# matwilso/generative_models

Measured on AMD Instinct MI355X. Metric: ddpm_train_images_per_sec, higher is better.
Workload: dtype fp16_fwd+bf16_bwd; 1 GPU; DDPM train step, 3x32x32, SimpleUnet C=128, 2048 images per GPU, T=1000 (BASELINE.json configs[2]); key=cfg2, global_batch=2048, parallelism=dp1

## Files before the change

generative_models_amd/csrc/conv1x1_stream.hip:

```cpp
#include <type_traits>

#include "gmk_common.h"

namespace {

constexpr int kRow = 272;

template <typename T>
__global__ __launch_bounds__(256) void conv1x1_pair_stream_kernel(const T* __restrict__ src, const T* __restrict__ w, T* __restrict__ out_a,
                                                                 T* __restrict__ out_b, unsigned npix, unsigned ntiles, unsigned src_bytes) {
    fp16_saturating_stores<T>();
    typedef typename Frag16<T>::type frag_t;
    typedef __attribute__((ext_vector_type(4))) unsigned int u32x4s;
    constexpr unsigned kBadOff = 0xFFFFFF00u;
    __shared__ __attribute__((aligned(16))) char wl[256 * kRow];
    __shared__ __attribute__((aligned(16))) char tile[128 * kRow];
    __shared__ __attribute__((aligned(16))) char trans[4 * 32 * kRow];
    const int tid = threadIdx.x, lane = tid & 63, wave = tid >> 6;
    const int r = lane & 31, h = lane >> 5;
    const __amdgpu_buffer_rsrc_t rss = __builtin_amdgcn_make_buffer_rsrc(const_cast<T*>(src), 0, (int)src_bytes, 0x00020000);
    const __amdgpu_buffer_rsrc_t rsa = __builtin_amdgcn_make_buffer_rsrc(out_a, 0, (int)src_bytes, 0x00020000);
    const __amdgpu_buffer_rsrc_t rsb = __builtin_amdgcn_make_buffer_rsrc(out_b, 0, (int)src_bytes, 0x00020000);
#pragma unroll
    for (int i = 0; i < 16; ++i) {
// ... 145 lines not shown
                s16x4 hi = __builtin_amdgcn_ds_read_tr16_b64_v4i16((GMK_LDS s16x4*)(Yb + (pxl + 4) * 256 + wa));
                const s16x8 t = {lo[0], lo[1], lo[2], lo[3], hi[0], hi[1], hi[2], hi[3]};
                a[i] = __builtin_bit_cast(bf16x8, t);
                lo = __builtin_amdgcn_ds_read_tr16_b64_v4i16((GMK_LDS s16x4*)(Xb + pxl * 256 + wb));
                hi = __builtin_amdgcn_ds_read_tr16_b64_v4i16((GMK_LDS s16x4*)(Xb + (pxl + 4) * 256 + wb));
                const s16x8 u = {lo[0], lo[1], lo[2], lo[3], hi[0], hi[1], hi[2], hi[3]};
                b[i] = __builtin_bit_cast(bf16x8, u);
            }
#pragma unroll
            for (int i = 0; i < 2; ++i)
#pragma unroll
                for (int j = 0; j < 2; ++j) acc[i][j] = __builtin_amdgcn_mfma_f32_32x32x16_bf16(a[i], b[j], acc[i][j], 0, 0, 0);
        }
        if (ks + 1 < nk) write_step(PAR ^ 1, ry[PAR ^ 1], rx0[PAR ^ 1], rx1[PAR ^ 1]);
        __syncthreads();
    };
    for (int ks = 0; ks < nk; ks += 2) {
        k_step(ks, std::integral_constant<int, 0>{});
        if (ks + 1 < nk) k_step(ks + 1, std::integral_constant<int, 1>{});
    }
    float* out = slab + (int64_t)blockIdx.x * (128 * 256) + cib * 128;
#pragma unroll
    for (int i = 0; i < 2; ++i)
#pragma unroll
        for (int j = 0; j < 2; ++j)
#pragma unroll
            for (int e = 0; e < 16; ++e) {
                const int co = wm * 64 + i * 32 + (e & 3) + 8 * (e >> 2) + 4 * h;
                const int ci = wn * 64 + j * 32 + r;
                out[co * 256 + ci] = acc[i][j][e];
            }
}

}

int gmk_conv1x1_pair_stream_try(const void* src, int64_t npix, const void* w_rows256, void* out_a, void* out_b, int dtype, hipStream_t stream) {
    if (!gmk_is16(dtype) || gmk_kernel_choice(3, "GMK_DEV_VARIANT") == 46) return 0;
    const int64_t bytes = npix * 256;
    if (bytes >= 0xFFFFFF00ll) return 0;
    const int64_t ntiles = (npix + 127) / 128;
    const int ncu = gmk_cu_limit();
    if (ntiles < 2 * ncu) return 0;
    const unsigned grid = (unsigned)ncu;
    if (dtype == GMK_BF16)
        conv1x1_pair_stream_kernel<bf16_t><<<grid, 256, 0, stream>>>((const bf16_t*)src, (const bf16_t*)w_rows256, (bf16_t*)out_a, (bf16_t*)out_b,
                                                                    (unsigned)npix, (unsigned)ntiles, (unsigned)bytes);
    else
        conv1x1_pair_stream_kernel<f16_t><<<grid, 256, 0, stream>>>((const f16_t*)src, (const f16_t*)w_rows256, (f16_t*)out_a, (f16_t*)out_b,
                                                                   (unsigned)npix, (unsigned)ntiles, (unsigned)bytes);
    return 1;
}

int gmk_conv1x1_wgrad_stream_try(const void* dy, int dy_cstride, const void* src0, const void* src1, int64_t npix, float* slab, int64_t slab_bytes,
                                 bool x_f16, hipStream_t stream) {
    if (gmk_kernel_choice(3, "GMK_DEV_VARIANT") == 47) return 0;
    const int ncu = gmk_cu_limit();
    if (npix < (int64_t)ncu * 64 * 8 || npix >= (1ll << 31) - 64) return 0;
    if (slab_bytes < (int64_t)ncu * 128 * 256 * 4) return 0;
    int64_t chunk = (npix + ncu - 1) / ncu;
    chunk = (chunk + 63) / 64 * 64;
    const int ns = (int)((npix + chunk - 1) / chunk);
    if (x_f16)
        conv1x1_wgrad_stream_kernel<f16_t><<<ns, 512, 0, stream>>>((const bf16_t*)dy, dy_cstride, (const f16_t*)src0, (const f16_t*)src1, slab, (int)npix, (int)chunk);
    else
        conv1x1_wgrad_stream_kernel<bf16_t><<<ns, 512, 0, stream>>>((const bf16_t*)dy, dy_cstride, (const bf16_t*)src0, (const bf16_t*)src1, slab, (int)npix, (int)chunk);
    return ns;
}
```

generative_models_amd/csrc/conv_igemm.hip:

```cpp
#include <stdlib.h>

#include <type_traits>

#include "gmk_common.h"

namespace {

constexpr int kBM = 128, kBN = 128;

struct GatherParams {
    int hs, ws;
    int ho, wo;
    int ksize, pad;
    int mul, shift, mask, lim_h, lim_w;
    signed char ty[9], tx[9];
    unsigned char tapw[9];
    int ntaps;
    int oscale, ooy, oox, out_w, out_hw;
};

__host__ bool make_gather(int mode, int ksize, int hs, int ws, int ho, int wo, GatherParams* g) {
    g->hs = hs; g->ws = ws; g->ho = ho; g->wo = wo;
    g->ksize = ksize; g->pad = ksize == 3 ? 1 : 0;
    g->mul = 1; g->shift = 0; g->mask = 0; g->lim_h = hs; g->lim_w = ws;
// ... 1120 lines not shown
            return gmk_check_launch("gmk_conv_wgrad(reduce)");
        }
    }
    if (wforce != 1 && ksize == 1 && mode == GMK_CONV_NORMAL && dtype == GMK_BF16 && c0 == 128 && c1 == 128 && cout == 128) {
        const int ns1 = gmk_conv1x1_wgrad_stream_try(dy, dy_cstride, src0, src1, (int64_t)B * ho * wo, (float*)workspace, workspace_bytes, xf16,
                                                     gmk_stream(stream));
        if (ns1 > 0) {
            gmk_note_kernel(15);
            int rc1 = gmk_check_launch("gmk_conv_wgrad(1x1 stream)");
            if (rc1) return rc1;
            launch_wgrad_reduce((const float*)workspace, dw, ns1, 1, cout, 256, gmk_stream(stream));
            return gmk_check_launch("gmk_conv_wgrad(reduce)");
        }
    }
    p.dy = dy; p.dy_cstride = dy_cstride; p.src0 = src0; p.src1 = src1; p.c0 = c0; p.c1 = c1; p.ktot = c0 + c1;
    p.cout = cout; p.M = B * ho * wo;
    const int ns = wgrad_nsplit(p.M, taps, cout, p.ktot, &p.chunk);
    const int64_t need = (int64_t)ns * taps * cout * p.ktot * 4;
    GMK_REQUIRE(workspace_bytes >= need, "gmk_conv_wgrad: workspace %lld < %lld bytes", (long long)workspace_bytes,
                (long long)need);
    p.slab = (float*)workspace;
    gmk_note_kernel(11);
    p.ns = ns; p.taps = taps; p.order = (gmk_kernel_choice(3, "GMK_DEV_VARIANT") & 0xFF) == 61;
    dim3 grid((ns + 7) / 8 * 8 * taps * (cout / 128) * (p.ktot / 128));
    if (dtype == GMK_BF16 && xf16) conv_wgrad_kernel<bf16_t, f16_t><<<grid, 256, 0, gmk_stream(stream)>>>(p);
    else if (dtype == GMK_BF16) conv_wgrad_kernel<bf16_t><<<grid, 256, 0, gmk_stream(stream)>>>(p);
    else if (fp32_split()) conv_wgrad_kernel<float, float, true><<<grid, 256, 0, gmk_stream(stream)>>>(p);
    else conv_wgrad_kernel<float><<<grid, 256, 0, gmk_stream(stream)>>>(p);
    int rc = gmk_check_launch("gmk_conv_wgrad");
    if (rc) return rc;
    launch_wgrad_reduce(p.slab, dw, ns, taps, cout, p.ktot, gmk_stream(stream));
    return gmk_check_launch("gmk_conv_wgrad(reduce)");
}
```

generative_models_amd/csrc/gmk_common.h:

```cpp
#pragma once
#include <hip/hip_runtime.h>
#include <stdint.h>

#include <type_traits>

#include "../../include/gmk.h"

typedef __bf16 bf16_t;
typedef __attribute__((ext_vector_type(8))) __bf16 bf16x8;
typedef __attribute__((ext_vector_type(4))) __bf16 bf16x4;
typedef _Float16 f16_t;
typedef __attribute__((ext_vector_type(8))) _Float16 f16x8;
typedef __attribute__((ext_vector_type(4))) _Float16 f16x4;
typedef __attribute__((ext_vector_type(2))) _Float16 f16x2;
typedef __attribute__((ext_vector_type(2))) __bf16 bf16x2;
typedef __attribute__((ext_vector_type(4))) short s16x4;
typedef __attribute__((ext_vector_type(4))) float f32x4;
typedef __attribute__((ext_vector_type(16))) float f32x16;

#define GMK_LDS __attribute__((address_space(3)))

void gmk_set_error(const char* fmt, ...);
int gmk_check_launch(const char* what);
int gmk_kernel_choice(int which, const char* env);
int gmk_conv1x1_pair_stream_try(const void* src, int64_t npix, const void* w_rows256, void* out_a, void* out_b, int dtype, hipStream_t stream);
int gmk_conv1x1_wgrad_stream_try(const void* dy, int dy_cstride, const void* src0, const void* src1, int64_t npix, float* slab, int64_t slab_bytes,
                                 bool x_f16, hipStream_t stream);
int gmk_conv_subpixel_takes(int B, int H, int W, int cin, int cout, int w_rows, int ntaps, int out_cstride, int dtype);
bool fp32_split(void);
int gmk_cu_limit(void);
void gmk_note_kernel(int id);

#define GMK_REQUIRE(cond, ...)                 \
    do {                                       \
        if (!(cond)) {                         \
            gmk_set_error(__VA_ARGS__);        \
            return GMK_ERR_ARG;                \
        }                                      \
    } while (0)

int gmk_conv3x3_halo_try(const void* src0, const void* src1, int c0, int c1, int B, int H, int W, const void* w, int w_rows,
                         int n0, int cout, const float* bias, const float* emb, int emb_stride, const void* residual,
                         void* out, int out_cstride, int min_tiles, int upsample, float* stats, int64_t stats_bytes,
                         const float* gn_scale, const float* gn_shift, int gn_stride, int dtype, hipStream_t stream);

struct HaloGeometry { int R, TP, slots; int64_t rows_total, M, ntiles, nb0, nb1, nbw, nbo; };
int gmk_halo_geometry(int B, int H, int W, int c0, int c1, int w_rows, int cout, int out_cstride, int min_tiles, int upsample,
                      int fused_gn, HaloGeometry* g);

int gmk_wgrad_slots_nsplit(int cout, int ktot);
int gmk_conv_wgrad_slots_try(const void* dy, int dy_cstride, const void* src0, const void* src1, int c0, int c1, int B, int H,
                             int W, int cout, float* slab, int64_t slab_bytes, int forced, int upsample, bool x_f16,
                             hipStream_t stream, int stride2 = 0);


static inline hipStream_t gmk_stream(void* s) { return reinterpret_cast<hipStream_t>(s); }
static inline int gmk_esize(int dtype) { return dtype == GMK_F32 ? 4 : 2; }
static inline bool gmk_is16(int dtype) { return dtype == GMK_BF16 || dtype == GMK_F16; }
template <typename T> struct gmk_tag { typedef T type; };
template <typename T> constexpr int gmk_dtype_of = std::is_same<T, float>::value ? GMK_F32 : std::is_same<T, bf16_t>::value ? GMK_BF16 : GMK_F16;
// ... 150 lines not shown
```

generative_models_amd/diffusion/simple_unet.py:

```python
import math
import os
from collections import OrderedDict

import torch
from torch import nn

from .. import ops

MAX_TIMESTEPS = 256


def _res_names(prefix, cin, cout, emb):
    out = [
        (f"{prefix}.in_layers.0.weight", (cin,)), (f"{prefix}.in_layers.0.bias", (cin,)),
        (f"{prefix}.in_layers.2.weight", (cout, cin, 3, 3)), (f"{prefix}.in_layers.2.bias", (cout,)),
        (f"{prefix}.emb_layers.1.weight", (cout, emb)), (f"{prefix}.emb_layers.1.bias", (cout,)),
        (f"{prefix}.out_layers.0.weight", (cout,)), (f"{prefix}.out_layers.0.bias", (cout,)),
        (f"{prefix}.out_layers.3.weight", (cout, cout, 3, 3)), (f"{prefix}.out_layers.3.bias", (cout,)),
    ]
    if cin != cout:
        out += [(f"{prefix}.skip_connection.weight", (cout, cin, 1, 1)), (f"{prefix}.skip_connection.bias", (cout,))]
    return out


# ... 538 lines not shown
                ops.set_cu_limit(part[0] - part[1])
        for t in tensors:
            t.record_stream(side)

    def _emb_ready(self):
        pend = getattr(self, "_emb_pending", None)
        if pend is not None:
            self._emb_pending = None
            self._join_side()
            pend.record_stream(torch.cuda.current_stream())

    def _join_side(self):
        if self._side is not None:
            torch.cuda.current_stream().wait_stream(self._side)

    def _res_bwd(self, name, ctx, dout, dout_sum, demb_all, blk, extra_add=None, grads=True, defer_skip=False):
        P, G, C = self._pv, self._gv, self.channels
        srcs, a, stats1, h, a2, (mean2, rstd2) = ctx.pop(name)
        B, H, W, _ = dout.shape
        two = len(srcs) == 2
        if grads:
            ops.colsum(dout_sum, G[f"{name}.out_layers.3.bias"], defer=True)
            self._wgrad(dout, [a2], 3, ops.NORMAL, G[f"{name}.out_layers.3.weight"])
        _, wd2 = self._packs[f"{name}.out_layers.3"]
        da2 = self._conv([dout], wd2, C, 3, ops.NORMAL, (H, W))
        dh, dgp, dbp = ops.gn_silu_bwd(da2, h, P[f"{name}.out_layers.0.weight"], P[f"{name}.out_layers.0.bias"], mean2,
                                       rstd2, dxsum=demb_all[:, blk * C:(blk + 1) * C] if grads else None,
                                       dropout=ctx.pop(name + ".dropout", None), xadd=ctx["emb_all"][:, blk * C:(blk + 1) * C])
        if grads:
            ops.colsum(dgp, G[f"{name}.out_layers.0.weight"], defer=True); ops.colsum(dbp, G[f"{name}.out_layers.0.bias"], defer=True)
            ops.colsum(demb_all[:, blk * C:(blk + 1) * C], G[f"{name}.in_layers.2.bias"], defer=True)
            self._wgrad(dh, a, 3, ops.NORMAL, G[f"{name}.in_layers.2.weight"])
        _, wd1 = self._packs[f"{name}.in_layers.2"]
        if two:
            if grads:
                ops.colsum(dout_sum, G[f"{name}.skip_connection.bias"], defer=True)
                self._wgrad(dout, srcs, 1, ops.NORMAL, G[f"{name}.skip_connection.weight"])
            _, wds = self._packs[f"{name}.skip_connection"]
        outs = []
        gw, gb = G[f"{name}.in_layers.0.weight"], G[f"{name}.in_layers.0.bias"]
        if two and C == 128:
            dskips = ops.conv1x1_pair(dout, wds, 2 * C)
        elif two:
            dskips = tuple(self._conv([dout], wds, 2 * C, 1, ops.NORMAL, (H, W), n0=i * C) for i in range(2))
        else:
            dskips = (dout,)
        for i, s in enumerate(srcs):
            da = self._conv([dh], wd1, len(srcs) * C, 3, ops.NORMAL, (H, W), n0=i * C)
            dskip = dskips[i]
            add2 = extra_add[i] if extra_add is not None else None
            gn = (da, dskip, P[f"{name}.in_layers.0.weight"][i * C:(i + 1) * C], P[f"{name}.in_layers.0.bias"][i * C:(i + 1) * C],
                  stats1[i][0], stats1[i][1])
            if defer_skip and i == 1 and grads and C == 128 and not self._narrow and ops.gn_pair_ok(s, self._g2, self._g1, da.dtype):
                outs.append((_DeferredGN(s, gn, gw[C:2 * C], gb[C:2 * C]), None))
                continue
            ssum = torch.empty((B, C), device=dout.device, dtype=torch.float32) if grads else None
            if isinstance(add2, _DeferredGN):
                assert add2.x is s
                ds, (ugp, ubp), (dgp, dbp) = ops.gn_silu_bwd_pair(s, add2.gn, gn, dxsum=ssum)
                ops.colsum(ugp, add2.gw, defer=True); ops.colsum(ubp, add2.gb, defer=True)
            else:
                ds, dgp, dbp = ops.gn_silu_bwd(da, s, *gn[2:], dadd1=dskip, dadd2=add2, dxsum=ssum)
            if grads:
                ops.colsum(dgp, gw[i * C:(i + 1) * C], defer=True); ops.colsum(dbp, gb[i * C:(i + 1) * C], defer=True)
            outs.append((ds, ssum))
        return outs

    def prepare_forward(self, dev=None):
        if self._packs_stale or self._packed_version != self._version_sum():
            self._repack()
        dev = self.flat_params.device if dev is None else dev
        self._freq_table(MAX_TIMESTEPS, dev)
        self._freq_table(4, dev)

# ... 189 lines not shown
```

generative_models_amd/ops.py:

```python
import math

import os

import torch

from ._lib import check, lib

F32, BF16, F16 = 0, 1, 2
_DT = {torch.float32: F32, torch.bfloat16: BF16, torch.float16: F16}
_HALF = (torch.bfloat16, torch.float16)
NORMAL, STRIDE2, UPSAMPLE2, TRANSPOSED2 = 0, 1, 2, 3

PROFILE = None


KERNEL_NAMES = {1: "conv_igemm_kernel", 2: "conv_igemm_dma_kernel", 3: "conv3x3_halo_kernel", 4: "conv3x3_halo_ws_kernel", 11: "conv_wgrad_kernel",
                12: "conv_wgrad_slots_kernel", 13: "conv_wgrad_slots_ws_kernel", 16: "conv_wgrad_subpixel_ws_kernel", 14: "conv1x1_pair_stream_kernel", 15: "conv1x1_wgrad_stream_kernel",
                5: "conv3x3_halo_ws_kernel[zero-stuffed transposed conv]",
                7: "conv3x3_halo_ws_kernel[+1x1 skip]",
                6: "conv_igemm_dma_kernel[stride-2 dgrad phases]",
                17: "conv_wgrad_slots_ws_kernel[stride-2 planes]",
                8: "conv_subpixel_ws_kernel[upsample]", 9: "conv_subpixel_ws_kernel[transposed]", 10: "conv_subpixel_ws_kernel[upsample dgrad]",
                21: "gn_silu_fwd_reg_kernel", 22: "gn_silu_fwd_kernel", 23: "gn_silu_bwd_hybrid_kernel", 24: "gn_silu_bwd_kernel",
                25: "gn_silu_bwd_pair_kernel", 26: "gn_silu_fwd_pair_kernel"}


def instantiation_key(name, dtype):
    if dtype not in _HALF:
        return None
    t = "f16" if dtype == torch.float16 else "bf16"
    if name == "conv3x3_halo_ws_kernel":
        return f"{name}<{t}>"
    if name == "conv3x3_halo_ws_kernel[+1x1 skip]":
        return f"conv3x3_halo_ws_kernel<{t},+skip>"
    if name == "conv_wgrad_slots_ws_kernel[stride-2 planes]":
        return "conv_wgrad_slots_ws_kernel<stride-2 planes>"
    if name.startswith("conv_subpixel_ws_kernel["):
        return f"conv_subpixel_ws_kernel<{t},{name[len('conv_subpixel_ws_kernel['):-1]}>"
    return None


def _nbytes(*tensors):
    if PROFILE is None:
        return 0.0
    return float(sum(t.numel() * t.element_size() for t in tensors if t is not None))


class _Timed:

    def __init__(self, name, flops, nbytes=0.0, fixed=False, multiplied=None, dtype=None):
# ... 88 lines not shown
    _f32(w, "w")
    cout, cin, k, _ = w.shape
    ref = w_fwd if w_fwd is not None else w_dgrad
    for t in (w_fwd, w_dgrad):
        if t is not None:
            _chk(t, name="pack")
            assert t.numel() == w.numel()
    if w_fwd is not None and w_dgrad is not None and w_fwd.dtype != w_dgrad.dtype:
        pack_conv_weight(w, w_fwd, None)
        pack_conv_weight(w, None, w_dgrad)
        return
    check(lib.gmk_pack_conv_weight(_p(w), _p(w_fwd), _p(w_dgrad), cout, cin, k, _DT[ref.dtype], _s()), "pack_conv_weight")


def pack_conv_weights_multi(arena, packs, table, fwd_f16=None):
    import ctypes
    _f32(arena, "arena"); _chk(packs, name="packs")
    n = len(table[0])
    arrs = [(ctypes.c_int * n)(*[int(v) for v in col]) for col in table]
    flags = (ctypes.c_int * n)(*[int(v) for v in fwd_f16]) if fwd_f16 is not None else None
    check(lib.gmk_pack_conv_weights_multi(_p(arena), _p(packs), n, *arrs, flags, _DT[packs.dtype], _s()), "pack_conv_weights_multi")


GN_STATS = False
GN_FUSE = os.environ.get("GMK_GN_FUSE", "1") != "0"
GN_FUSE_MIN_HW = int(os.environ.get("GMK_GN_FUSE_MIN_HW", "2048"))
SKIP_FOLD = os.environ.get("GMK_SKIP_FOLD", "1") != "0"
SKIP_FOLD_OVER_FUSE = os.environ.get("GMK_SKIP_FOLD_FUSE", "fold") != "fuse"
EMB_SIDE = os.environ.get("GMK_EMB_SIDE", "1") == "1"
FWD_SIDE = os.environ.get("GMK_FWD_SIDE", "0") == "1"
WGRAD_CUS = int(os.environ.get("GMK_WGRAD_CUS", "0"))
WGRAD_STREAM = os.environ.get("GMK_WGRAD_STREAM", "1") != "0"
GN_PAIR = os.environ.get("GMK_GN_PAIR", "1") != "0"


def _xadd_stride(xadd, B, C):
    if xadd is None:
        return 0
    assert xadd.dtype == torch.float32 and xadd.shape == (B, C) and xadd.stride(1) == 1 and xadd.is_cuda
    return xadd.stride(0)


def gn_silu_fwd(x, gamma, beta, groups, eps=1e-5, dropout=None, xadd=None):
    _chk(x, name="x"); _f32(gamma, "gamma"); _f32(beta, "beta")
    B, H, W, C = x.shape
    assert gamma.numel() == C and beta.numel() == C
    y = torch.empty_like(x)
    ncol = groups if groups > 0 else (C - groups - 1) // -groups
    mean = torch.empty((B, ncol), device=x.device, dtype=torch.float32)
    rstd = torch.empty_like(mean)
    mean._gn_groups = groups
    st = getattr(x, "_gn_stats", None)
    part, tp, nt = st if st is not None else (None, 0, 0)
    dp, dseed, doff = dropout if dropout is not None else (0.0, 0, 0)
    xs = _xadd_stride(xadd, B, C)
    with _Timed("gn_silu_fwd", 0.0, _nbytes(x, y)):
        check(lib.gmk_gn_silu_fwd(_p(x), _p(y), _p(gamma), _p(beta), _p(mean), _p(rstd), B, H * W, C, groups, eps, _p(part), tp, nt,
                                  float(dp), int(dseed), int(doff), _p(xadd), xs, _DT[x.dtype], _s()), "gn_silu_fwd")
    return y, mean, rstd


def gn_stats(x, gamma, beta, groups, tab_scale, tab_shift, eps=1e-5, xadd=None):
    _chk(x, name="x"); _f32(gamma, "gamma"); _f32(beta, "beta")
    assert x.dtype in _HALF
    B, H, W, C = x.shape
    for t in (tab_scale, tab_shift):
# ... 262 lines not shown
    B, H, W, c0 = src.shape
    return skips[0].shape[3] == skips[1].shape[3] and bool(lib.gmk_conv3x3_skipfold_ok(B, H, W, c0, skips[0].shape[3], 128))


def conv3x3_skipfold(src, w, bias, skips, wsk, bias_sk, cout=128):
    s0 = _chk(src, name="src")
    k0, k1 = _chk(skips[0], s0.dtype, "skip0"), _chk(skips[1], s0.dtype, "skip1")
    B, H, W, c0 = s0.shape
    cs = k0.shape[3]
    assert k0.shape == k1.shape == (B, H, W, cs)
    _chk(w, s0.dtype, "w"); _chk(wsk, s0.dtype, "wsk")
    assert w.numel() == 9 * cout * c0 and wsk.numel() == cout * 2 * cs, (w.numel(), wsk.numel())
    _f32(bias, "bias"); _f32(bias_sk, "bias_sk")
    assert bias.numel() == cout and bias_sk.numel() == cout
    out = torch.empty((B, H, W, cout), device=s0.device, dtype=s0.dtype)
    with _Timed("conv_igemm", 2.0 * B * H * W * cout * (9 * c0 + 2 * cs), _nbytes(s0, k0, k1, out), dtype=s0.dtype):
        check(lib.gmk_conv3x3_skipfold(_p(s0), c0, B, H, W, _p(w), cout, 0, cout, _p(bias), _p(k0), _p(k1), cs, _p(wsk), cout, 0,
                                       _p(bias_sk), _p(out), cout, _DT[s0.dtype], _s()), "conv3x3_skipfold")
    return out


def conv1x1_pair(src, w, w_rows, n0=0):
    s0 = _chk(src, name="src")
    B, H, W, c = s0.shape
    _chk(w, s0.dtype, "w")
    assert w.numel() == w_rows * c and n0 + 256 <= w_rows
    oa = torch.empty((B, H, W, 128), device=s0.device, dtype=s0.dtype)
    ob = torch.empty_like(oa)
    with _Timed("conv_igemm", 2.0 * B * H * W * 256 * c, _nbytes(s0, oa, ob)):
        check(lib.gmk_conv1x1_pair(_p(s0), c, B, H, W, _p(w), w_rows, n0, _p(oa), _p(ob), _DT[s0.dtype], _s()), "conv1x1_pair")
    return oa, ob


_WS = {}


def _workspace(nbytes, device, tag="conv"):
    key = (tag, device.index, _s())
    ws = _WS.get(key)
    if ws is None or ws.numel() < nbytes:
        ws = torch.empty(int(nbytes), device=device, dtype=torch.uint8)
        _WS[key] = ws
    return ws


def conv_wgrad(dy, srcs, ksize, mode, dw):
    _chk(dy, name="dy")
    s0 = _chk(srcs[0], name="src0")
    s1 = _chk(srcs[1], s0.dtype, "src1") if len(srcs) > 1 else None
    assert s0.dtype == dy.dtype or (s0.dtype == torch.float16 and dy.dtype == torch.bfloat16), (s0.dtype, dy.dtype)
    B, hs, ws_, c0 = s0.shape
    c1 = s1.shape[3] if s1 is not None else 0
    _, ho, wo, cout = dy.shape
    assert dy.shape[0] == B
    assert dw.dtype == torch.float32 and dw.is_contiguous() and dw.numel() == cout * (c0 + c1) * ksize * ksize
    need = lib.gmk_conv_wgrad_workspace_bytes(B * ho * wo, ksize * ksize, cout, c0 + c1)
    assert need > 0
    wsbuf = _workspace(need, dy.device)
    with _Timed("conv_wgrad", 2.0 * B * ho * wo * cout * (c0 + c1) * ksize * ksize, _nbytes(dy, s0, s1)):
        check(lib.gmk_conv_wgrad(_p(dy), cout, _p(s0), _p(s1), c0, c1, B, hs, ws_, ho, wo, ksize, mode, _p(dw), cout,
                                 _p(wsbuf), wsbuf.numel(), _DT[dy.dtype], _DT[s0.dtype], _s()), "conv_wgrad")
    return dw


def conv_wgrad_subpixel_ok(B, H, W, c, dy_dtype, cout=128):
    return dy_dtype == torch.bfloat16 and bool(lib.gmk_conv_wgrad_subpixel_ok(B, H, W, c, cout))
# ... 633 lines not shown
```

include/gmk.h:

```cpp
#ifndef GMK_H
#define GMK_H
#include <stdint.h>

#ifdef __cplusplus
extern "C" {
#endif

#define GMK_F32 0
#define GMK_BF16 1
#define GMK_F16 2
#define GMK_ERR_ARG (-1)

#define GMK_CONV_NORMAL 0
#define GMK_CONV_STRIDE2 1
#define GMK_CONV_UPSAMPLE2 2
#define GMK_CONV_TRANSPOSED2 3

int gmk_version(void);
const char* gmk_last_error(void);
int gmk_last_kernel(void);
int gmk_set_kernel_choice(int conv, int wgrad, int gn);
int gmk_set_dev_variant(int v);
int gmk_dev_set_stamp_buffer(void* buf, int64_t bytes);
int gmk_set_cu_limit(int n);
// ... 11 lines not shown
                    int B, int HW, int C, int groups, float eps, const float* stats_part, int tile_pixels, int ntiles,
                    float drop_p, uint64_t drop_seed, uint64_t drop_offset, const float* xadd, int xadd_stride, int dtype,
                    void* stream);
int gmk_gn_silu_bwd(const void* dy, const void* x, const float* gamma, const float* beta, const float* mean,
                    const float* rstd, const void* dadd1, const void* dadd2, void* dx, float* dgamma_part,
                    float* dbeta_part, float* dxsum, int dxsum_stride, int B, int HW, int C, int groups,
                    float drop_p, uint64_t drop_seed, uint64_t drop_offset, const float* xadd, int xadd_stride, int dtype,
                    int x_dtype, void* stream);
int gmk_gn_pair_ok(int HW, int C, int groups_a, int groups_b, int x_dtype, int grad_dtype);
int gmk_gn_pair_fwd_ok(int HW, int C, int groups_a, int groups_b, int dtype);
int gmk_gn_silu_fwd_pair(const void* x, void* y_a, void* y_b, const float* gamma_a, const float* beta_a, const float* gamma_b,
                         const float* beta_b, float* mean_a, float* rstd_a, float* mean_b, float* rstd_b, int B, int HW, int C,
                         int groups_a, int groups_b, float eps, const float* xadd, int xadd_stride, int dtype, void* stream);
int gmk_gn_silu_bwd_pair(const void* x, const void* dy_up, const void* dadd_up, const float* gamma_up, const float* beta_up,
                         const float* mean_up, const float* rstd_up, float* dgamma_part_up, float* dbeta_part_up, int groups_up,
                         const void* dy_dn, const void* dadd_dn, const float* gamma_dn, const float* beta_dn, const float* mean_dn,
                         const float* rstd_dn, float* dgamma_part_dn, float* dbeta_part_dn, int groups_dn, void* dx, float* dxsum,
                         int dxsum_stride, int B, int HW, int C, const float* xadd, int xadd_stride, int x_dtype, void* stream);
int gmk_cast16(const void* src, void* dst, int64_t n, int src_dtype, int dst_dtype, void* stream);
int gmk_chansum(const void* x, float* out, int out_stride, int B, int HW, int C, int dtype, void* stream);
int gmk_colsum(const float* part, int64_t stride, float* out, int R, int C, int accumulate, void* stream);
int gmk_colsum_multi(int n, const float* const* part, const int64_t* stride, float* const* out, const int* R,
                     const int* C, void* stream);
int gmk_sumpool2x2(const void* x, void* y, int B, int H, int W, int C, int dtype, void* stream);

int gmk_conv_igemm(const void* src0, const void* src1, int c0, int c1, int B, int hs, int ws, int ho, int wo,
                   int ksize, int mode, const void* w, int w_rows, int n0, int cout, const float* bias,
                   const float* emb, int emb_stride, const void* residual, void* out, int out_cstride,
                   float* gn_stats, int64_t gn_stats_bytes, const float* gn_scale, const float* gn_shift, int gn_stride,
                   int dtype, void* stream);
int gmk_conv_gn_fusable(int B, int H, int W, int c0, int c1, int cout);
int gmk_conv1x1_pair(const void* src, int c, int B, int H, int W, const void* w, int w_rows, int n0, void* out_a, void* out_b,
                     int dtype, void* stream);
int gmk_conv3x3_skipfold_ok(int B, int H, int W, int c0, int cs, int cout);
int gmk_conv3x3_skipfold(const void* src, int c0, int B, int H, int W, const void* w, int w_rows, int n0, int cout,
                         const float* bias, const void* sk0, const void* sk1, int cs, const void* wsk, int wsk_rows, int nsk0,
                         const float* bias_sk, void* out, int out_cstride, int dtype, void* stream);
#define GMK_SUBPIXEL_UPSAMPLE 0
#define GMK_SUBPIXEL_TRANSPOSED 1
#define GMK_SUBPIXEL_UPSAMPLE_DGRAD 2
int gmk_conv_subpixel_ok(int B, int H, int W, int cin, int cout, int dtype);
int gmk_pack_upsample_weight(const float* w, void* w_sub, void* w_sub_dgrad, int cout, int cin, int dtype, int dgrad_dtype, void* stream);
int gmk_conv_subpixel(const void* src, int B, int H, int W, int cin, const void* w, int w_rows, int n0, int cout, int mode,
                      const float* bias, const void* residual, void* out, int out_cstride, int dtype, void* stream);
int gmk_conv_wgrad_subpixel_ok(int B, int H, int W, int cin, int cout);
int64_t gmk_conv_wgrad_subpixel_workspace_bytes(int B, int H, int W, int cin, int cout);
int gmk_conv_wgrad_subpixel(const void* dy, int dy_cstride, const void* x, int B, int H, int W, int cin, int cout, float* dw,
                            void* workspace, int64_t workspace_bytes, int dtype, int x_dtype, void* stream);
int gmk_gn_stats(const void* x, const float* gamma, const float* beta, float* mean, float* rstd, float* tab_scale,
                 float* tab_shift, int tab_stride, int B, int HW, int C, int groups, float eps, const float* xadd,
                 int xadd_stride, int dtype, void* stream);
int gmk_conv_wgrad(const void* dy, int dy_cstride, const void* src0, const void* src1, int c0, int c1, int B,
                   int hs, int ws, int ho, int wo, int ksize, int mode, float* dw, int cout, void* workspace,
                   int64_t workspace_bytes, int dtype, int x_dtype, void* stream);

int gmk_stem_fwd(const float* x, const float* w, const float* bias, void* y, int B, int cin, int H, int W, int C,
                 int dtype, void* stream);
int gmk_stem_wgrad_blocks(int64_t n_pixels);
int gmk_stem_wgrad(const float* x, const void* dy, float* dw_part, int B, int cin, int H, int W, int C, int dtype,
                   void* stream);
int gmk_head_fwd(const void* a, const float* w, const float* bias, float* out, int B, int cout, int H, int W, int C,
                 int dtype, void* stream);
int gmk_head_dgrad(const float* dout, const float* w, void* da, int B, int cout, int H, int W, int C, int dtype,
                   void* stream);
int gmk_head_wgrad_blocks(int64_t n_pixels);
int gmk_head_wgrad(const float* dout, const void* a, float* dw_part, int B, int cout, int H, int W, int C, int dtype,
// ... 87 lines not shown
```

Before: 46530 images/s.

## Fuse 1x1 skip-connection weight gradient and input gradient into one streaming kernel

```diff
diff --git a/generative_models_amd/csrc/conv1x1_stream.hip b/generative_models_amd/csrc/conv1x1_stream.hip
--- a/generative_models_amd/csrc/conv1x1_stream.hip
+++ b/generative_models_amd/csrc/conv1x1_stream.hip
@@ -201,6 +201,167 @@
             }
 }
 
+template <typename TX>
+__global__ __launch_bounds__(512) void conv1x1_skip_bwd_stream_kernel(const bf16_t* __restrict__ dy, int dy_cstride, const TX* __restrict__ src0,
+                                                                     const TX* __restrict__ src1, const bf16_t* __restrict__ w, bf16_t* __restrict__ out_a,
+                                                                     bf16_t* __restrict__ out_b, float* __restrict__ slab, int M, int chunk,
+                                                                     unsigned out_bytes) {
+    typedef __attribute__((ext_vector_type(4))) unsigned int u32x4s;
+    typedef __attribute__((ext_vector_type(8))) short s16x8;
+    constexpr unsigned kBadOff = 0xFFFFFF00u;
+    __shared__ __attribute__((aligned(16))) char smem[2 * 3 * 16384];
+    __shared__ __attribute__((aligned(16))) char trans[2 * 64 * kRow];
+    const int tid = threadIdx.x, lane = tid & 63, wave = tid >> 6;
+    const int wm = wave >> 2, wq = wave & 3, cib = wq >> 1, wn = wq & 1;
+    const int pix_begin = blockIdx.x * chunk;
+    const int pix_end = min(pix_begin + chunk, M);
+    const int nk = pix_end > pix_begin ? (pix_end - pix_begin + 63) / 64 : 0;
+    const __amdgpu_buffer_rsrc_t rsa = __builtin_amdgcn_make_buffer_rsrc(out_a, 0, (int)out_bytes, 0x00020000);
+    const __amdgpu_buffer_rsrc_t rsb = __builtin_amdgcn_make_buffer_rsrc(out_b, 0, (int)out_bytes, 0x00020000);
+    int lds_w[2], srow[2];
+    const int sc = tid & 15;
+#pragma unroll
+    for (int j = 0; j < 2; ++j) {
+        const int row = (tid >> 4) + 32 * j;
+        srow[j] = row;
+        lds_w[j] = row * 256 + ((((sc >> 2) ^ (row & 3)) << 2 | (sc & 3)) << 4);
+    }
+    u32x4s ry[2][2], rx0[2][2], rx1[2][2];
+    auto load_step = [&](int ks, u32x4s (&y)[2], u32x4s (&x0)[2], u32x4s (&x1)[2]) {
+#pragma unroll
+        for (int j = 0; j < 2; ++j) {
+            const int m = pix_begin + ks * 64 + srow[j];
+            u32x4s vy = {0u, 0u, 0u, 0u}, v0 = vy, v1 = vy;
+            if (m < pix_end) {
+                vy = *reinterpret_cast<const u32x4s*>(dy + (int64_t)m * dy_cstride + sc * 8);
+                v0 = *reinterpret_cast<const u32x4s*>(src0 + (int64_t)m * 128 + sc * 8);
+                v1 = *reinterpret_cast<const u32x4s*>(src1 + (int64_t)m * 128 + sc * 8);
+            }
+            y[j] = vy; x0[j] = v0; x1[j] = v1;
+        }
+    };
+    auto round_x = [&](u32x4s v) {
+        if constexpr (!__is_same(TX, bf16_t)) {
+#pragma unroll
+            for (int d = 0; d < 4; ++d) {
+                float lo, hi;
+                unpack_pair<TX>(v[d], lo, hi);
+                v[d] = pack_pair<bf16_t>(lo, hi);
+            }
+        }
+        return v;
+    };
+    auto write_step = [&](int buf, const u32x4s (&y)[2], const u32x4s (&x0)[2], const u32x4s (&x1)[2]) {
+        char* b = smem + buf * 49152;
+#pragma unroll
+        for (int j = 0; j < 2; ++j) {
+            *reinterpret_cast<u32x4s*>(b + lds_w[j]) = y[j];
+            *reinterpret_cast<u32x4s*>(b + 16384 + lds_w[j]) = round_x(x0[j]);
+            *reinterpret_cast<u32x4s*>(b + 32768 + lds_w[j]) = round_x(x1[j]);
+        }
+    };
+    f32x16 acc[2][2];
+#pragma unroll
+    for (int i = 0; i < 2; ++i)
+#pragma unroll
+        for (int j = 0; j < 2; ++j)
+#pragma unroll
+            for (int e = 0; e < 16; ++e) acc[i][j][e] = 0.f;
+    const int gg = lane >> 4, i16 = lane & 15, q = i16 >> 2, pp = i16 & 3;
+    const int hh = gg >> 1, cblk = gg & 1;
+    const int r = lane & 31, h = lane >> 5;
+    bf16x8 wf[8];
+#pragma unroll
+    for (int kk = 0; kk < 8; ++kk) wf[kk] = *reinterpret_cast<const bf16x8*>(w + (wave * 32 + r) * 128 + 16 * kk + 8 * h);
+    if (nk > 0) {
+        load_step(0, ry[0], rx0[0], rx1[0]);
+        if (nk > 1) load_step(1, ry[1], rx0[1], rx1[1]);
+        write_step(0, ry[0], rx0[0], rx1[0]);
+    }
+    __syncthreads();
+    auto k_step = [&](int ks, auto par) {
+        constexpr int PAR = decltype(par)::value;
+        if (ks + 2 < nk) load_step(ks + 2, ry[PAR], rx0[PAR], rx1[PAR]);
+        const char* Yb = smem + PAR * 49152;
+        const char* Xb = Yb + 16384 + cib * 16384;
+#pragma unroll
+        for (int kk = 0; kk < 4; ++kk) {
+            bf16x8 a[2], b[2];
+            const int pxl = kk * 16 + 8 * hh + q;
+#pragma unroll
+            for (int i = 0; i < 2; ++i) {
+                const int wa = (((wm * 2 + i) ^ q) << 6) + 32 * cblk + 8 * pp;
+                const int wb = (((wn * 2 + i) ^ q) << 6) + 32 * cblk + 8 * pp;
+                s16x4 lo = __builtin_amdgcn_ds_read_tr16_b64_v4i16((GMK_LDS s16x4*)(Yb + pxl * 256 + wa));
+                s16x4 hi = __builtin_amdgcn_ds_read_tr16_b64_v4i16((GMK_LDS s16x4*)(Yb + (pxl + 4) * 256 + wa));
+                const s16x8 t = {lo[0], lo[1], lo[2], lo[3], hi[0], hi[1], hi[2], hi[3]};
+                a[i] = __builtin_bit_cast(bf16x8, t);
+                lo = __builtin_amdgcn_ds_read_tr16_b64_v4i16((GMK_LDS s16x4*)(Xb + pxl * 256 + wb));
+                hi = __builtin_amdgcn_ds_read_tr16_b64_v4i16((GMK_LDS s16x4*)(Xb + (pxl + 4) * 256 + wb));
+                const s16x8 u = {lo[0], lo[1], lo[2], lo[3], hi[0], hi[1], hi[2], hi[3]};
+                b[i] = __builtin_bit_cast(bf16x8, u);
+            }
+#pragma unroll
+            for (int i = 0; i < 2; ++i)
+#pragma unroll
+                for (int j = 0; j < 2; ++j) acc[i][j] = __builtin_amdgcn_mfma_f32_32x32x16_bf16(a[i], b[j], acc[i][j], 0, 0, 0);
+        }
+#pragma unroll
+        for (int pb = 0; pb < 2; ++pb) {
+            const int row = pb * 32 + r;
+            f32x16 d;
+#pragma unroll
+            for (int e = 0; e < 16; ++e) d[e] = 0.f;
+#pragma unroll
+            for (int kk = 0; kk < 8; ++kk) {
+                const bf16x8 bfr = *reinterpret_cast<const bf16x8*>(Yb + row * 256 + (((((kk >> 1) ^ (row & 3)) << 2) | (2 * (kk & 1) + h)) << 4));
+                d = __builtin_amdgcn_mfma_f32_32x32x16_bf16(wf[kk], bfr, d, 0, 0, 0);
+            }
+            unsigned pk[4][2];
+#pragma unroll
+            for (int q4 = 0; q4 < 4; ++q4) {
+                pk[q4][0] = pack_pair<bf16_t>(d[4 * q4], d[4 * q4 + 1]);
+                pk[q4][1] = pack_pair<bf16_t>(d[4 * q4 + 2], d[4 * q4 + 3]);
+            }
+            char* trow = trans + wm * (64 * kRow) + row * kRow + wq * 64;
+#pragma unroll
+            for (int q4 = 0; q4 < 4; q4 += 2) {
+                const auto s0 = __builtin_amdgcn_permlane32_swap(pk[q4][0], pk[q4 + 1][0], false, false);
+                const auto s1 = __builtin_amdgcn_permlane32_swap(pk[q4][1], pk[q4 + 1][1], false, false);
+                const u32x4s o = {s0[0], s1[0], s0[1], s1[1]};
+                *reinterpret_cast<u32x4s*>(trow + (q4 + h) * 16) = o;
+            }
+        }
+        if (ks + 1 < nk) write_step(PAR ^ 1, ry[PAR ^ 1], rx0[PAR ^ 1], rx1[PAR ^ 1]);
+        __syncthreads();
+        u32x4s v[4];
+        const int orow = ((tid >> 4) & 31);
+#pragma unroll
+        for (int j = 0; j < 4; ++j) v[j] = *reinterpret_cast<const u32x4s*>(trans + (j >> 1) * (64 * kRow) + (orow + 32 * (j & 1)) * kRow + sc * 16);
+        __syncthreads();
+#pragma unroll
+        for (int j = 0; j < 4; ++j) {
+            const int m = pix_begin + ks * 64 + orow + 32 * (j & 1);
+            __builtin_amdgcn_raw_buffer_store_b128(v[j], (j >> 1) ? rsb : rsa, m < pix_end ? (unsigned)m * 256u + (unsigned)sc * 16u : kBadOff, 0, 0);
+        }
+    };
+    for (int ks = 0; ks < nk; ks += 2) {
+        k_step(ks, std::integral_constant<int, 0>{});
+        if (ks + 1 < nk) k_step(ks + 1, std::integral_constant<int, 1>{});
+    }
+    float* out = slab + (int64_t)blockIdx.x * (128 * 256) + cib * 128;
+#pragma unroll
+    for (int i = 0; i < 2; ++i)
+#pragma unroll
+        for (int j = 0; j < 2; ++j)
+#pragma unroll
+            for (int e = 0; e < 16; ++e) {
+                const int co = wm * 64 + i * 32 + (e & 3) + 8 * (e >> 2) + 4 * h;
+                const int ci = wn * 64 + j * 32 + r;
+                out[co * 256 + ci] = acc[i][j][e];
+            }
+}
+
 }
 
 int gmk_conv1x1_pair_stream_try(const void* src, int64_t npix, const void* w_rows256, void* out_a, void* out_b, int dtype, hipStream_t stream) {
@@ -235,3 +396,23 @@
         conv1x1_wgrad_stream_kernel<bf16_t><<<ns, 512, 0, stream>>>((const bf16_t*)dy, dy_cstride, (const bf16_t*)src0, (const bf16_t*)src1, slab, (int)npix, (int)chunk);
     return ns;
 }
+
+int gmk_conv1x1_skip_bwd_stream_try(const void* dy, int dy_cstride, const void* src0, const void* src1, int64_t npix, const void* w_rows256,
+                                    void* out_a, void* out_b, float* slab, int64_t slab_bytes, bool x_f16, int force, hipStream_t stream) {
+    const int variant = gmk_kernel_choice(3, "GMK_DEV_VARIANT");
+    if (variant == 46 || variant == 47) return -1;
+    const int ncu = gmk_cu_limit();
+    if (!force && npix < (int64_t)ncu * 64 * 8) return -1;
+    if (npix <= 0 || npix * 256 >= 0xFFFFFF00ll) return 0;
+    int64_t chunk = (npix + ncu - 1) / ncu;
+    chunk = (chunk + 63) / 64 * 64;
+    const int ns = (int)((npix + chunk - 1) / chunk);
+    if (slab_bytes < (int64_t)ns * 128 * 256 * 4) return 0;
+    if (x_f16)
+        conv1x1_skip_bwd_stream_kernel<f16_t><<<ns, 512, 0, stream>>>((const bf16_t*)dy, dy_cstride, (const f16_t*)src0, (const f16_t*)src1, (const bf16_t*)w_rows256,
+                                                                      (bf16_t*)out_a, (bf16_t*)out_b, slab, (int)npix, (int)chunk, (unsigned)(npix * 256));
+    else
+        conv1x1_skip_bwd_stream_kernel<bf16_t><<<ns, 512, 0, stream>>>((const bf16_t*)dy, dy_cstride, (const bf16_t*)src0, (const bf16_t*)src1, (const bf16_t*)w_rows256,
+                                                                       (bf16_t*)out_a, (bf16_t*)out_b, slab, (int)npix, (int)chunk, (unsigned)(npix * 256));
+    return ns;
+}
diff --git a/generative_models_amd/csrc/conv_igemm.hip b/generative_models_amd/csrc/conv_igemm.hip
--- a/generative_models_amd/csrc/conv_igemm.hip
+++ b/generative_models_amd/csrc/conv_igemm.hip
@@ -1176,3 +1176,42 @@
     launch_wgrad_reduce(p.slab, dw, ns, taps, cout, p.ktot, gmk_stream(stream));
     return gmk_check_launch("gmk_conv_wgrad(reduce)");
 }
+
+extern "C" int gmk_conv1x1_skip_bwd_ok(int B, int H, int W) {
+    const int variant = gmk_kernel_choice(3, "GMK_DEV_VARIANT");
+    const int64_t npix = (int64_t)B * H * W;
+    return B > 0 && H > 0 && W > 0 && variant != 46 && variant != 47 && gmk_kernel_choice(1, "GMK_WGRAD_KERNEL") != 1 &&
+           npix >= (int64_t)gmk_cu_limit() * 64 * 8 && npix * 256 < 0xFFFFFF00ll;
+}
+
+extern "C" int gmk_conv1x1_skip_bwd(const void* dy, int dy_cstride, const void* src0, const void* src1, int B, int H, int W, const void* w,
+                                    int w_rows, int n0, void* out_a, void* out_b, float* dw, void* workspace, int64_t workspace_bytes,
+                                    int x_dtype, int force, void* stream) {
+    GMK_REQUIRE(dy && src0 && src1 && w && out_a && out_b && workspace, "gmk_conv1x1_skip_bwd: null pointer");
+    GMK_REQUIRE(n0 >= 0 && n0 + 256 <= w_rows, "gmk_conv1x1_skip_bwd: rows n0 .. n0 + 255 outside the %d packed rows", w_rows);
+    GMK_REQUIRE(x_dtype == GMK_BF16 || x_dtype == GMK_F16, "gmk_conv1x1_skip_bwd: sources of type %d (bf16 or fp16 beside the bf16 gradient)", x_dtype);
+    GMK_REQUIRE(dy_cstride >= 128 && dy_cstride % 8 == 0, "gmk_conv1x1_skip_bwd: gradient channel stride %d", dy_cstride);
+    GMK_REQUIRE(B > 0 && H > 0 && W > 0, "gmk_conv1x1_skip_bwd: empty problem");
+    GMK_REQUIRE(force || gmk_conv1x1_skip_bwd_ok(B, H, W), "gmk_conv1x1_skip_bwd: %d x %d x %d is not a problem of the streaming kernel (gmk_conv1x1_skip_bwd_ok)", B, H, W);
+    const int ns = gmk_conv1x1_skip_bwd_stream_try(dy, dy_cstride, src0, src1, (int64_t)B * H * W, (const char*)w + (size_t)n0 * 128 * 2, out_a, out_b,
+                                                   (float*)workspace, workspace_bytes, x_dtype == GMK_F16, force, gmk_stream(stream));
+    GMK_REQUIRE(ns > 0, "gmk_conv1x1_skip_bwd: not launched (%d): workspace of %lld bytes too small, results beyond 4 GiB or a development switch", ns,
+                (long long)workspace_bytes);
+    gmk_note_kernel(18);
+    int rc = gmk_check_launch("gmk_conv1x1_skip_bwd");
+    if (rc || !dw) return rc;
+    return gmk_conv1x1_skip_bwd_reduce(workspace, ns, dw, stream);
+}
+
+extern "C" int gmk_conv1x1_skip_bwd_slabs(int B, int H, int W) {
+    const int64_t npix = (int64_t)B * H * W, ncu = gmk_cu_limit();
+    if (npix <= 0) return 0;
+    const int64_t chunk = ((npix + ncu - 1) / ncu + 63) / 64 * 64;
+    return (int)((npix + chunk - 1) / chunk);
+}
+
+extern "C" int gmk_conv1x1_skip_bwd_reduce(const void* workspace, int nslabs, float* dw, void* stream) {
+    GMK_REQUIRE(workspace && dw && nslabs > 0 && nslabs <= 256, "gmk_conv1x1_skip_bwd_reduce: bad arguments (%d slabs)", nslabs);
+    launch_wgrad_reduce((const float*)workspace, dw, nslabs, 1, 128, 256, gmk_stream(stream));
+    return gmk_check_launch("gmk_conv1x1_skip_bwd(reduce)");
+}
diff --git a/generative_models_amd/csrc/gmk_common.h b/generative_models_amd/csrc/gmk_common.h
--- a/generative_models_amd/csrc/gmk_common.h
+++ b/generative_models_amd/csrc/gmk_common.h
@@ -26,6 +26,8 @@
 int gmk_conv1x1_pair_stream_try(const void* src, int64_t npix, const void* w_rows256, void* out_a, void* out_b, int dtype, hipStream_t stream);
 int gmk_conv1x1_wgrad_stream_try(const void* dy, int dy_cstride, const void* src0, const void* src1, int64_t npix, float* slab, int64_t slab_bytes,
                                  bool x_f16, hipStream_t stream);
+int gmk_conv1x1_skip_bwd_stream_try(const void* dy, int dy_cstride, const void* src0, const void* src1, int64_t npix, const void* w_rows256,
+                                    void* out_a, void* out_b, float* slab, int64_t slab_bytes, bool x_f16, int force, hipStream_t stream);
 int gmk_conv_subpixel_takes(int B, int H, int W, int cin, int cout, int w_rows, int ntaps, int out_cstride, int dtype);
 bool fp32_split(void);
 int gmk_cu_limit(void);
diff --git a/generative_models_amd/diffusion/simple_unet.py b/generative_models_amd/diffusion/simple_unet.py
--- a/generative_models_amd/diffusion/simple_unet.py
+++ b/generative_models_amd/diffusion/simple_unet.py
@@ -594,14 +594,19 @@
             ops.colsum(demb_all[:, blk * C:(blk + 1) * C], G[f"{name}.in_layers.2.bias"], defer=True)
             self._wgrad(dh, a, 3, ops.NORMAL, G[f"{name}.in_layers.2.weight"])
         _, wd1 = self._packs[f"{name}.in_layers.2"]
+        fused = False
         if two:
+            _, wds = self._packs[f"{name}.skip_connection"]
+            fused = C == 128 and wds.dtype == dout.dtype and ops.conv1x1_skip_bwd_ok(dout, srcs, grads)
             if grads:
                 ops.colsum(dout_sum, G[f"{name}.skip_connection.bias"], defer=True)
-                self._wgrad(dout, srcs, 1, ops.NORMAL, G[f"{name}.skip_connection.weight"])
-            _, wds = self._packs[f"{name}.skip_connection"]
+                if not fused:
+                    self._wgrad(dout, srcs, 1, ops.NORMAL, G[f"{name}.skip_connection.weight"])
         outs = []
         gw, gb = G[f"{name}.in_layers.0.weight"], G[f"{name}.in_layers.0.bias"]
-        if two and C == 128:
+        if fused:
+            dskips = ops.conv1x1_skip_bwd(dout, srcs, wds, 2 * C, G[f"{name}.skip_connection.weight"], reduce_on=self._on_side)
+        elif two and C == 128:
             dskips = ops.conv1x1_pair(dout, wds, 2 * C)
         elif two:
             dskips = tuple(self._conv([dout], wds, 2 * C, 1, ops.NORMAL, (H, W), n0=i * C) for i in range(2))
diff --git a/generative_models_amd/ops.py b/generative_models_amd/ops.py
--- a/generative_models_amd/ops.py
+++ b/generative_models_amd/ops.py
@@ -16,6 +16,7 @@
 
 KERNEL_NAMES = {1: "conv_igemm_kernel", 2: "conv_igemm_dma_kernel", 3: "conv3x3_halo_kernel", 4: "conv3x3_halo_ws_kernel", 11: "conv_wgrad_kernel",
                 12: "conv_wgrad_slots_kernel", 13: "conv_wgrad_slots_ws_kernel", 16: "conv_wgrad_subpixel_ws_kernel", 14: "conv1x1_pair_stream_kernel", 15: "conv1x1_wgrad_stream_kernel",
+                18: "conv1x1_skip_bwd_stream_kernel",
                 5: "conv3x3_halo_ws_kernel[zero-stuffed transposed conv]",
                 7: "conv3x3_halo_ws_kernel[+1x1 skip]",
                 6: "conv_igemm_dma_kernel[stride-2 dgrad phases]",
@@ -170,6 +171,7 @@
 WGRAD_CUS = int(os.environ.get("GMK_WGRAD_CUS", "0"))
 WGRAD_STREAM = os.environ.get("GMK_WGRAD_STREAM", "1") != "0"
 GN_PAIR = os.environ.get("GMK_GN_PAIR", "1") != "0"
+SKIP_BWD_FUSED = os.environ.get("GMK_SKIP_BWD_FUSED", "1") != "0"
 
 
 def _xadd_stride(xadd, B, C):
@@ -498,6 +500,45 @@
     return oa, ob
 
 
+def conv1x1_skip_bwd_ok(dout, srcs, grads=True):
+    if not (SKIP_BWD_FUSED and grads and len(srcs) == 2 and dout.dtype == torch.bfloat16 and dout.shape[3] == 128):
+        return False
+    if not all(s.dtype in _HALF and s.dtype == srcs[0].dtype and s.shape == dout.shape for s in srcs):
+        return False
+    B, H, W, _ = dout.shape
+    return bool(lib.gmk_conv1x1_skip_bwd_ok(B, H, W))
+
+
+def conv1x1_skip_bwd(dout, srcs, w, w_rows, dw, n0=0, force=False, reduce_on=None):
+    if not dout.is_cuda or dout.dtype != torch.bfloat16 or dout.dim() != 4 or dout.shape[3] != 128:
+        raise ValueError("dout: expected a bf16 device tensor [B, H, W, 128]")
+    B, H, W, _ = dout.shape
+    cs = dout.stride(2)
+    if dout.stride() != (H * W * cs, W * cs, cs, 1) or cs < 128 or cs % 8 or dout.data_ptr() % 16:
+        raise ValueError(f"dout: strides {dout.stride()} are not those of a 16-byte aligned channel block of a contiguous NHWC tensor")
+    s0 = _chk(srcs[0], name="src0")
+    s1 = _chk(srcs[1], s0.dtype, "src1")
+    assert s0.dtype in _HALF and s0.shape == s1.shape == (B, H, W, 128), (s0.dtype, s0.shape, s1.shape)
+    _chk(w, torch.bfloat16, "w")
+    assert w.numel() == w_rows * 128 and 0 <= n0 and n0 + 256 <= w_rows
+    assert dw.dtype == torch.float32 and dw.is_contiguous() and dw.numel() == 128 * 256
+    oa = torch.empty((B, H, W, 128), device=dout.device, dtype=dout.dtype)
+    ob = torch.empty_like(oa)
+    ns = lib.gmk_conv1x1_skip_bwd_slabs(B, H, W)
+    slabs = torch.empty((max(ns, 1), 128 * 256), device=dout.device, dtype=torch.float32)
+    npix = B * H * W
+    nbytes = 5.0 * npix * 256 + 2.0 * slabs.numel() * 4 if PROFILE is not None else 0.0
+    with _Timed("conv1x1_skip_bwd", 2.0 * npix * 128 * 256 * 2, nbytes):
+        check(lib.gmk_conv1x1_skip_bwd(_p(dout), cs, _p(s0), _p(s1), B, H, W, _p(w), w_rows, n0, _p(oa), _p(ob), None, _p(slabs), slabs.numel() * 4,
+                                       _DT[s0.dtype], int(bool(force)), _s()), "conv1x1_skip_bwd")
+    reduce = lambda: check(lib.gmk_conv1x1_skip_bwd_reduce(_p(slabs), ns, _p(dw), _s()), "conv1x1_skip_bwd_reduce")
+    if reduce_on is None:
+        reduce()
+    else:
+        reduce_on(reduce, (slabs,))
+    return oa, ob
+
+
 _WS = {}
 
 
diff --git a/include/gmk.h b/include/gmk.h
--- a/include/gmk.h
+++ b/include/gmk.h
@@ -67,6 +67,12 @@
 int gmk_conv_gn_fusable(int B, int H, int W, int c0, int c1, int cout);
 int gmk_conv1x1_pair(const void* src, int c, int B, int H, int W, const void* w, int w_rows, int n0, void* out_a, void* out_b,
                      int dtype, void* stream);
+int gmk_conv1x1_skip_bwd_ok(int B, int H, int W);
+int gmk_conv1x1_skip_bwd_slabs(int B, int H, int W);
+int gmk_conv1x1_skip_bwd_reduce(const void* workspace, int nslabs, float* dw, void* stream);
+int gmk_conv1x1_skip_bwd(const void* dy, int dy_cstride, const void* src0, const void* src1, int B, int H, int W, const void* w,
+                         int w_rows, int n0, void* out_a, void* out_b, float* dw, void* workspace, int64_t workspace_bytes,
+                         int x_dtype, int force, void* stream);
 int gmk_conv3x3_skipfold_ok(int B, int H, int W, int c0, int cs, int cout);
 int gmk_conv3x3_skipfold(const void* src, int c0, int B, int H, int W, const void* w, int w_rows, int n0, int cout,
                          const float* bias, const void* sk0, const void* sk1, int cs, const void* wsk, int wsk_rows, int nsk0,
```

Measured after the change: 46930 images/s, median of 6. No clear change (+0.8%).
